# lukecq1231/nats

Measured on AMD Instinct MI355X. Metric: train_tokens_per_sec, higher is better.
Workload: dtype bf16; 1 GPU; model=distraction-gru-seq2seq, dim=1000, dim_word=100, enc_depth=1, dim_att=100, vocab=30000, src_len=800, tgt_len=100, batch_per_gpu=20, global_batch=20, seq_len=800, optimizer=adadelta+clip100, parallelism=dp1, step_graph=False

## Files before the change

### nats_amd/ops/hip/cond_gru.hip

```cpp

#include <torch/extension.h>
#include <ATen/cuda/CUDAContext.h>

#include <algorithm>

#include "common.h"
#include "gru_kernels.h"

namespace {

__global__ void cond_small_gemm_bt(const bf16_t* __restrict__ A,
                                   const bf16_t* __restrict__ Bt,
                                   float* __restrict__ Cpart, int B, int N,
                                   int ldK, int Kpad) {
  const int m0 = blockIdx.x * 16;
  const int n0 = blockIdx.y * 16;
  const int KS = gridDim.z;
  const int kchunk = ((Kpad / KS + 31) / 32) * 32;
  const int kbeg = min(Kpad, (int)blockIdx.z * kchunk);
  const int kend = min(Kpad, kbeg + kchunk);
  f32x4 acc = {0.f, 0.f, 0.f, 0.f};
  NATS_MFMA_KLOOP(acc, A, m0, ldK, Bt, n0, Kpad, kbeg, kend);
  const int lane = threadIdx.x & (NATS_WAVE - 1);
  const int col = n0 + (lane & 15);
  const int rbase = m0 + (lane >> 4) * 4;
  if (col >= N) return;
  float* C = Cpart + (long)blockIdx.z * 32 * N;
#pragma unroll
  for (int i = 0; i < 4; ++i) {
    const int row = rbase + i;
    if (row < B) C[(long)row * N + col] = acc[i];
  }
}

__global__ __launch_bounds__(256) void cond_attn_escore(
    const float* __restrict__ pctx,
    const float* __restrict__ ps_part,
    int PS_KS,
    const float* __restrict__ accA,
    const float* __restrict__ Dwei,
    const float* __restrict__ Uatt,
    const float* __restrict__ catt_p,
    float* __restrict__ e_buf,
    int B, int Ts, int A) {
  extern __shared__ float sm_e[];
  float* sm_ps = sm_e;
  float* sm_dw = sm_e + A;
  float* sm_ua = sm_e + 2 * A;
  const int b = blockIdx.x;
  for (int i = threadIdx.x; i < A; i += blockDim.x) {
    float ps = 0.f;
    for (int k = 0; k < PS_KS; ++k) ps += ps_part[((long)k * 32 + b) * A + i];
    sm_ps[i] = ps;
    sm_dw[i] = Dwei[i];
    sm_ua[i] = Uatt[i];
  }
  __syncthreads();
  const int s = blockIdx.y * blockDim.x + threadIdx.x;
  if (s >= Ts) return;
  const int ACH = gridDim.z;
  const int chunkA = ((A + ACH - 1) / ACH + 3) & ~3;
  const int ibeg = blockIdx.z * chunkA;
  const int iend = min(A, ibeg + chunkA);
  if (ibeg >= iend) return;
  const float accAu = accA[(long)b * Ts + s];
  const float* prow = pctx + ((long)s * B + b) * A;
  float e = (blockIdx.z == 0) ? catt_p[0] : 0.f;
  for (int i = ibeg; i < iend; ++i) {
    e += tanhf(prow[i] + sm_ps[i] + accAu * sm_dw[i]) * sm_ua[i];
  }
  if (ACH == 1) {
    e_buf[(long)s * B + b] += e;
  } else {
    atomicAdd(e_buf + (long)s * B + b, e);
  }
}

__global__ __launch_bounds__(1024) void cond_attn_softmax(
    float* __restrict__ accA,
    float* __restrict__ accA_used_t,
    const float* __restrict__ ctx_mask,
    const float* __restrict__ mask_t,
    float* __restrict__ e_buf,
    float* __restrict__ alphas_t,
    const float* __restrict__ ps_part,
    int PS_KS,
    float* __restrict__ pstate_t,
    int A,
    int B, int Ts) {
  {
    const int b0 = blockIdx.x;
    for (int i = threadIdx.x; i < A; i += blockDim.x) {
      float ps = 0.f;
      for (int k = 0; k < PS_KS; ++k)
        ps += ps_part[((long)k * 32 + b0) * A + i];
      pstate_t[(long)b0 * A + i] = ps;
    }
  }
  const int b = blockIdx.x;

  float lmax = -INFINITY;
  for (int s = threadIdx.x; s < Ts; s += blockDim.x) {
    if (ctx_mask != nullptr && ctx_mask[(long)s * B + b] == 0.f) continue;
    lmax = fmaxf(lmax, e_buf[(long)s * B + b]);
  }
  const float bmax = block_reduce_max(lmax);
  const float M = isfinite(bmax) ? bmax : 0.f;

  float lsum = 0.f;
  for (int s = threadIdx.x; s < Ts; s += blockDim.x) {
    float a = __expf(e_buf[(long)s * B + b] - M);
    e_buf[(long)s * B + b] = 0.f;
    if (ctx_mask != nullptr) a *= ctx_mask[(long)s * B + b];
    alphas_t[(long)b * Ts + s] = a;
    lsum += a;
  }
  const float inv = 1.f / block_reduce_sum(lsum);

  const float mm = (mask_t != nullptr) ? mask_t[b] : 1.f;
  for (int s = threadIdx.x; s < Ts; s += blockDim.x) {
    const float al = alphas_t[(long)b * Ts + s] * inv;
    alphas_t[(long)b * Ts + s] = al;
    accA_used_t[(long)b * Ts + s] = accA[(long)b * Ts + s];
    accA[(long)b * Ts + s] += mm * al;
  }
}

__global__ void cond_attn_ctx_partial(
    const bf16_t* __restrict__ ctx_bf,
    const float* __restrict__ alphas_t,
    float* __restrict__ ctxpre_f32,
    int B, int Ts, int C, int SCH) {
  const int b = blockIdx.x;
  const int c = blockIdx.y * blockDim.x + threadIdx.x;
  if (c >= C) return;
  const int chunk = (Ts + SCH - 1) / SCH;
  const int sbeg = blockIdx.z * chunk;
  const int send = min(Ts, sbeg + chunk);
  float s0 = 0.f, s1 = 0.f, s2 = 0.f, s3 = 0.f;
  int s = sbeg;
  for (; s + 4 <= send; s += 4) {
    s0 += (float)ctx_bf[((long)(s + 0) * B + b) * C + c] *
          alphas_t[(long)b * Ts + s + 0];
    s1 += (float)ctx_bf[((long)(s + 1) * B + b) * C + c] *
          alphas_t[(long)b * Ts + s + 1];
    s2 += (float)ctx_bf[((long)(s + 2) * B + b) * C + c] *
          alphas_t[(long)b * Ts + s + 2];
    s3 += (float)ctx_bf[((long)(s + 3) * B + b) * C + c] *
          alphas_t[(long)b * Ts + s + 3];
  }
  for (; s < send; ++s)
    s0 += (float)ctx_bf[((long)s * B + b) * C + c] *
          alphas_t[(long)b * Ts + s];
  atomicAdd(&ctxpre_f32[(long)b * C + c], s0 + s1 + s2 + s3);
}

__global__ void cond_attn_gate_fwd(
    float* __restrict__ ctxpre_f32,
    const float* __restrict__ Ucon, const float* __restrict__ Wcon,
    float* __restrict__ accC,
    bf16_t* __restrict__ accC_used_t,
    bf16_t* __restrict__ ctxpre_t,
    float* __restrict__ ctxs_t,
    bf16_t* __restrict__ hc_bf,
    int ctx_off, int ldK1, const float* __restrict__ mask_t, int B, int C) {
  const int b = blockIdx.x;
  const int c = blockIdx.y * blockDim.x + threadIdx.x;
  if (c >= C) return;
  const float sum = ctxpre_f32[(long)b * C + c];
  ctxpre_f32[(long)b * C + c] = 0.f;
  ctxpre_t[(long)b * C + c] = (bf16_t)sum;
  const float accCv = accC[(long)b * C + c];
  accC_used_t[(long)b * C + c] = (bf16_t)accCv;
  const float g = tanhf(Ucon[c] * sum + accCv * Wcon[c]);
  ctxs_t[(long)b * C + c] = g;
  hc_bf[(long)b * ldK1 + ctx_off + c] = (bf16_t)g;
  const float mm = (mask_t != nullptr) ? mask_t[b] : 1.f;
  accC[(long)b * C + c] = accCv + mm * g;
}

__global__ __launch_bounds__(1024) void cond_gru1_step_fwd(
    const bf16_t* __restrict__ hc_bf,
    const float* __restrict__ h1_t,
    const bf16_t* __restrict__ W1pk,
    const float* __restrict__ b1,
    const float* __restrict__ bx1,
    const float* __restrict__ mask_t,
    float* __restrict__ h2_t,
    bf16_t* __restrict__ h2bf_out,
    int ld_h2bf,
    float* __restrict__ saved1_t,
    int B, int H, int K1) {
  __shared__ float pre[4][2][32][JB + 1];

  const int wg = blockIdx.x;
  const int wave = threadIdx.x / NATS_WAVE;
  const int m = wave / 8;
  const int g = (wave % 8) / 2;
  const int ks = wave % 2;
  const int j0 = wg * JB;
  const int khalf = ((K1 / 2 + 31) / 32) * 32;
  const int kbeg = ks * khalf;
  const int kend = min(K1, (ks + 1) * khalf);

  f32x4 acc = {0.f, 0.f, 0.f, 0.f};
  const bf16_t* brow = W1pk + (long)(wg * 4 + g) * JB * K1;
  NATS_MFMA_KLOOP(acc, hc_bf, 16 * m, K1, brow, 0, K1, kbeg, kend);
  store_cd_lds(pre[g][ks], acc, 16 * m);
  __syncthreads();

  for (int idx = threadIdx.x; idx < B * JB; idx += blockDim.x) {
    const int b = idx / JB;
    const int c = idx % JB;
    const int j = j0 + c;
    if (j >= H) continue;
    const float pxa = pre[2][0][b][c] + pre[2][1][b][c];
    const float pxb = pre[3][0][b][c] + pre[3][1][b][c];
    const GruCellFwd o = gru_cell_fwd(
        pre[0][0][b][c] + pre[0][1][b][c] + b1[j],
        pre[1][0][b][c] + pre[1][1][b][c] + b1[H + j], pxa + bx1[j], pxb,
        h1_t[(long)b * H + j], mask_t, b);
    h2_t[(long)b * H + j] = o.hnew;
    h2bf_out[(long)b * ld_h2bf + j] = (bf16_t)o.hnew;
    saved1_t[(long)b * 4 * H + j] = o.r;
    saved1_t[(long)b * 4 * H + H + j] = o.u;
    saved1_t[(long)b * 4 * H + 2 * H + j] = pxa;
    saved1_t[(long)b * 4 * H + 3 * H + j] = o.hbar;
  }
}

__global__ __launch_bounds__(1024) void cond_gru1_gemm_splitk(
    const bf16_t* __restrict__ hc_bf,
    const bf16_t* __restrict__ W1pk,
    float* __restrict__ part,
    int H, int K1, int Hpad) {
  __shared__ float pre[4][2][32][JB + 1];

  const int wg = blockIdx.x;
  const int ksb = blockIdx.y;
  const int KS = gridDim.y;
  const int wave = threadIdx.x / NATS_WAVE;
  const int m = wave / 8;
  const int g = (wave % 8) / 2;
  const int ks = wave % 2;
  const int j0 = wg * JB;
  const int nchunk = 2 * KS;
  const int kchunk = ((K1 / nchunk + 31) / 32) * 32;
  const int kidx = 2 * ksb + ks;
  const int kbeg = min(K1, kidx * kchunk);
  const int kend = min(K1, (kidx + 1) * kchunk);

  f32x4 acc = {0.f, 0.f, 0.f, 0.f};
  const bf16_t* brow = W1pk + (long)(wg * 4 + g) * JB * K1;
  NATS_MFMA_KLOOP(acc, hc_bf, 16 * m, K1, brow, 0, K1, kbeg, kend);
  store_cd_lds(pre[g][ks], acc, 16 * m);
  __syncthreads();

  float* dst = part + ((long)ksb * 4 + 0) * 32 * Hpad;
  for (int idx = threadIdx.x; idx < 4 * 32 * JB; idx += blockDim.x) {
    const int gg = idx / (32 * JB);
    const int b = (idx / JB) % 32;
    const int c = idx % JB;
    dst[((long)gg * 32 + b) * Hpad + j0 + c] =
        pre[gg][0][b][c] + pre[gg][1][b][c];
  }
}

__global__ void cond_gru1_step_pointwise(
    const float* __restrict__ part,
    int KS,
    const float* __restrict__ h1_t,
    const float* __restrict__ b1,
    const float* __restrict__ bx1,
    const float* __restrict__ mask_t,
    float* __restrict__ h2_t,
    bf16_t* __restrict__ h2bf_out,
    int ld_h2bf,
    float* __restrict__ saved1_t,
    int B, int H, int Hpad) {
  const long total = (long)B * H;
  for (long idx = blockIdx.x * blockDim.x + threadIdx.x; idx < total;
       idx += (long)gridDim.x * blockDim.x) {
    const int b = idx / H;
    const int j = idx % H;
    float p0 = 0.f, p1 = 0.f, p2 = 0.f, p3 = 0.f;
    const long bj = (long)b * Hpad + j;
    for (int k = 0; k < KS; ++k) {
      const float* pk = part + (long)k * 4 * 32 * Hpad;
      p0 += pk[bj];
      p1 += pk[(long)32 * Hpad + bj];
      p2 += pk[(long)2 * 32 * Hpad + bj];
      p3 += pk[(long)3 * 32 * Hpad + bj];
    }
    const float pxa = p2;
    const GruCellFwd o = gru_cell_fwd(p0 + b1[j], p1 + b1[H + j],
                                      pxa + bx1[j], p3, h1_t[idx], mask_t, b);
    h2_t[idx] = o.hnew;
    h2bf_out[(long)b * ld_h2bf + j] = (bf16_t)o.hnew;
    saved1_t[(long)b * 4 * H + j] = o.r;
    saved1_t[(long)b * 4 * H + H + j] = o.u;
    saved1_t[(long)b * 4 * H + 2 * H + j] = pxa;
    saved1_t[(long)b * 4 * H + 3 * H + j] = o.hbar;
  }
}


__global__ void cond_gru1_bwd_pointwise(
    const float* __restrict__ dh_carry,
    const float* __restrict__ dh_carry2,
    const float* __restrict__ dh2_all_t,
    const float* __restrict__ saved1_t,
    const float* __restrict__ h1_all_t,
    const float* __restrict__ bx1,
    const float* __restrict__ mask_t,
    bf16_t* __restrict__ dstep1,
    bf16_t* __restrict__ dstepC,
    int ldK3,
    float* __restrict__ ddirect_h1,
    bf16_t* __restrict__ dpre1_t,
    const float* __restrict__ dctxs_t,
    const float* __restrict__ daccC,
    float* __restrict__ dctx_dir,
    int C,
    float* __restrict__ dot_buf,
    int B, int H) {
  const long total = (long)B * H;
  const long total_all = total + (long)B * C + B;
  for (long idx2 = blockIdx.x * blockDim.x + threadIdx.x; idx2 < total_all;
       idx2 += (long)gridDim.x * blockDim.x) {
    if (idx2 >= total) {
      const long e = idx2 - total;
      if (e < (long)B * C) {
        const int b = e / C;
        const float mm = (mask_t != nullptr) ? mask_t[b] : 1.f;
        float v = mm * daccC[e];
        if (dctxs_t != nullptr) v += dctxs_t[e];
        dctx_dir[e] = v;
      } else {
        dot_buf[e - (long)B * C] = 0.f;
      }
      continue;
    }
    const long idx = idx2;
    const int b = idx / H;
    const int j = idx % H;
    float dh2 = dh_carry[idx];
    if (dh_carry2 != nullptr) dh2 += dh_carry2[idx];
    if (dh2_all_t != nullptr) dh2 += dh2_all_t[idx];
    const float r2 = saved1_t[(long)b * 4 * H + j];
    const float u2 = saved1_t[(long)b * 4 * H + H + j];
    const float pxa = saved1_t[(long)b * 4 * H + 2 * H + j];
    const float hbar = saved1_t[(long)b * 4 * H + 3 * H + j];
    const float h1v = h1_all_t[idx];
    const float mm = (mask_t != nullptr) ? mask_t[b] : 1.f;
    const GruCellBwd o =
        gru_cell_bwd(dh2, r2, u2, pxa + bx1[j], hbar, h1v, mm);
    ddirect_h1[idx] = o.ddirect;
    dstep1[(long)b * ldK3 + j] = (bf16_t)o.dpr;
    dstep1[(long)b * ldK3 + H + j] = (bf16_t)o.dpu;
    dstep1[(long)b * ldK3 + 2 * H + j] = (bf16_t)o.dpxl;
    dstepC[(long)b * ldK3 + j] = (bf16_t)o.dpr;
    dstepC[(long)b * ldK3 + H + j] = (bf16_t)o.dpu;
    dstepC[(long)b * ldK3 + 2 * H + j] = (bf16_t)o.dpx;
    dpre1_t[(long)b * 4 * H + j] = (bf16_t)o.dpr;
    dpre1_t[(long)b * 4 * H + H + j] = (bf16_t)o.dpu;
    dpre1_t[(long)b * 4 * H + 2 * H + j] = (bf16_t)o.dpx;
    dpre1_t[(long)b * 4 * H + 3 * H + j] = (bf16_t)o.dpxl;
  }
}

__global__ __launch_bounds__(384) void cond_bwd_gemm_dual_gate(
    const bf16_t* __restrict__ dstep1, const bf16_t* __restrict__ U1cat,
    const float* __restrict__ ddirect_h1, float* __restrict__ dh1_buf,
    int H, const bf16_t* __restrict__ dstepC,
    const bf16_t* __restrict__ W1cat, const float* __restrict__ dctx_dir,
    int C, int Kpad,
    const float* __restrict__ ctxs_t,
    const float* __restrict__ Ucon, const float* __restrict__ Wcon,
    float* __restrict__ daccC,
    float* __restrict__ dctxpre_f32,
    bf16_t* __restrict__ dctxpre_all_t,
    const bf16_t* __restrict__ ctxpre_t,
    const bf16_t* __restrict__ accC_used_t,
    float* __restrict__ gdUcon,
    float* __restrict__ gdWcon,
    int B) {
  __shared__ float ucon_s[JB], wcon_s[JB];
  __shared__ float part[3][32][JB + 1];
  const bool ctx_side = (blockIdx.y == 1);
  if (ctx_side && threadIdx.x < JB) {
    ucon_s[threadIdx.x] = 0.f;
    wcon_s[threadIdx.x] = 0.f;
  }
  const int N = ctx_side ? C : H;
  if ((int)blockIdx.x * JB >= N) return;
  const bf16_t* dstep = ctx_side ? dstepC : dstep1;
  const bf16_t* Wt = ctx_side ? W1cat : U1cat;

  const int wg = blockIdx.x;
  const int wave = threadIdx.x / NATS_WAVE;
  const int m = wave / 3;
  const int ks = wave % 3;
  const int i0 = wg * JB;
  const int kchunk = ((Kpad / 3 + 31) / 32) * 32;
  const int kbeg = ks * kchunk;
  const int kend = min(Kpad, (ks + 1) * kchunk);
  f32x4 acc = {0.f, 0.f, 0.f, 0.f};
  NATS_MFMA_KLOOP(acc, dstep, 16 * m, Kpad, Wt, i0, Kpad, kbeg, kend);
  store_cd_lds(part[ks], acc, 16 * m);
  __syncthreads();

  for (int idx = threadIdx.x; idx < B * JB; idx += blockDim.x) {
    const int b = idx / JB;
    const int cc = idx % JB;
    const int i = i0 + cc;
    if (i >= N) continue;
    const long bi = (long)b * N + i;
    const float sum = part[0][b][cc] + part[1][b][cc] + part[2][b][cc];
    if (!ctx_side) {
      dh1_buf[bi] = ddirect_h1[bi] + sum;
    } else {
      const float v = dctx_dir[bi] + sum;
      const float g = ctxs_t[bi];
      const float dg = v * (1.f - g * g);
      const float dpre = dg * Ucon[i];
      dctxpre_f32[bi] = dpre;
      dctxpre_all_t[bi] = (bf16_t)dpre;
      daccC[bi] += dg * Wcon[i];
      atomicAdd(ucon_s + cc, dg * (float)ctxpre_t[bi]);
      atomicAdd(wcon_s + cc, dg * (float)accC_used_t[bi]);
    }
  }
  if (ctx_side) {
    __syncthreads();
    if (threadIdx.x < JB && i0 + (int)threadIdx.x < N) {
      atomicAdd(gdUcon + i0 + threadIdx.x, ucon_s[threadIdx.x]);
      atomicAdd(gdWcon + i0 + threadIdx.x, wcon_s[threadIdx.x]);
    }
  }
}

__device__ __forceinline__ bf16x8 frag_a_f32pad(const float* A, int row0,
                                                int ld, int k0, int Rows,
                                                int Kcols) {
  const int lane = threadIdx.x & (NATS_WAVE - 1);
  const int r = row0 + (lane & 15);
  const int kb = k0 + (lane >> 4) * 8;
  bf16x8 v;
#pragma unroll
  for (int i = 0; i < 8; ++i) {
    const int k = kb + i;
    v[i] = (bf16_t)((r < Rows && k < Kcols) ? A[(long)r * ld + k] : 0.f);
  }
  return v;
}

__global__ __launch_bounds__(384) void cond_dh_carry_gemm_split(
    const bf16_t* __restrict__ dstep,
    const bf16_t* __restrict__ Wt,
    const float* __restrict__ ddirect,
    float* __restrict__ out,
    int B, int H, int Kpad) {
  __shared__ float part[3][32][JB + 1];
  const int wg = blockIdx.x;
  const int ks2 = blockIdx.y;
  const int wave = threadIdx.x / NATS_WAVE;
  const int m = wave / 3;
  const int ks = wave % 3;
  const int i0 = wg * JB;
  const int khalf = ((Kpad / 2 + 31) / 32) * 32;
  const int hbeg = min(Kpad, ks2 * khalf);
  const int hend = min(Kpad, hbeg + khalf);
  const int kchunk = (((hend - hbeg) / 3 + 31) / 32) * 32;
  const int kbeg = hbeg + ks * kchunk;
  const int kend = min(hend, kbeg + kchunk);
  f32x4 acc = {0.f, 0.f, 0.f, 0.f};
  NATS_MFMA_KLOOP(acc, dstep, 16 * m, Kpad, Wt, i0, Kpad, kbeg, kend);
  store_cd_lds(part[ks], acc, 16 * m);
  __syncthreads();
  float* o = out + (long)ks2 * B * H;
  for (int idx = threadIdx.x; idx < B * JB; idx += blockDim.x) {
    const int b = idx / JB;
    const int cc = idx % JB;
    const int i = i0 + cc;
    if (i >= H) continue;
    float v = part[0][b][cc] + part[1][b][cc] + part[2][b][cc];
    if (ks2 == 0) v += ddirect[(long)b * H + i];
    o[(long)b * H + i] = v;
  }
}

__global__ __launch_bounds__(384) void cond_dh1_att_gemm(
    const float* __restrict__ dpstate_t,
    const bf16_t* __restrict__ WattB,
    float* __restrict__ dh1_buf,
    int B, int H, int A, int Apad) {
  __shared__ float part[3][32][JB + 1];
  const int wg = blockIdx.x;
  const int wave = threadIdx.x / NATS_WAVE;
  const int m = wave / 3;
  const int ks = wave % 3;
  const int i0 = wg * JB;
  const int kchunk = ((Apad / 3 + 31) / 32) * 32;
  const int kbeg = ks * kchunk;
  const int kend = min(Apad, (ks + 1) * kchunk);
  f32x4 acc = {0.f, 0.f, 0.f, 0.f};
  for (int k = kbeg; k + 32 <= kend; k += 32) {
    bf16x8 a = frag_a_f32pad(dpstate_t, 16 * m, A, k, B, A);
    bf16x8 bfr = frag_bt_rowmajor(WattB, i0, Apad, k);
    acc = __builtin_amdgcn_mfma_f32_16x16x32_bf16(a, bfr, acc, 0, 0, 0);
  }
  store_cd_lds(part[ks], acc, 16 * m);
  __syncthreads();
  for (int idx = threadIdx.x; idx < B * JB; idx += blockDim.x) {
    const int b = idx / JB;
    const int cc = idx % JB;
    const int i = i0 + cc;
    if (i >= H) continue;
    dh1_buf[(long)b * H + i] +=
        part[0][b][cc] + part[1][b][cc] + part[2][b][cc];
  }
}

__global__ __launch_bounds__(256) void cond_attn_bwd_dalpha(
    const bf16_t* __restrict__ ctx_bf,
    const float* __restrict__ dctxpre_f32,
    const float* __restrict__ alphas_t,
    const float* __restrict__ daccA,
    const float* __restrict__ mask_t,
    const float* __restrict__ dalphas_t,
    float* __restrict__ dal_buf,
    float* __restrict__ dot_buf,
    int B, int Ts, int C) {
  const int b = blockIdx.x;
  const int wave = threadIdx.x / NATS_WAVE;
  const int lane = threadIdx.x & (NATS_WAVE - 1);
  const int s = blockIdx.y * 4 + wave;
  if (s >= Ts) return;
  const bf16_t* crow = ctx_bf + ((long)s * B + b) * C;
  const float* drow = dctxpre_f32 + (long)b * C;
  float part = 0.f;
  const int C8 = C & ~7;
  for (int c = lane * 8; c < C8; c += NATS_WAVE * 8) {
    bf16x8 v = *(const bf16x8*)(crow + c);
    const float4 d0 = *(const float4*)(drow + c);
    const float4 d1 = *(const float4*)(drow + c + 4);
    part += (float)v[0] * d0.x + (float)v[1] * d0.y + (float)v[2] * d0.z +
            (float)v[3] * d0.w + (float)v[4] * d1.x + (float)v[5] * d1.y +
            (float)v[6] * d1.z + (float)v[7] * d1.w;
  }
  for (int c = C8 + lane; c < C; c += NATS_WAVE) {
    part += (float)crow[c] * drow[c];
  }
#pragma unroll
  for (int off = NATS_WAVE / 2; off > 0; off >>= 1)
    part += __shfl_down(part, off);
  if (lane == 0) {
    float dal = part;
    const float mm = (mask_t != nullptr) ? mask_t[b] : 1.f;
    dal += mm * daccA[(long)b * Ts + s];
    if (dalphas_t != nullptr) dal += dalphas_t[(long)b * Ts + s];
    dal_buf[(long)s * B + b] = dal;
  }
}

__global__ __launch_bounds__(256) void cond_attn_bwd_dot(
    const float* __restrict__ alphas_t, const float* __restrict__ dal_buf,
    float* __restrict__ dot_buf, int B, int Ts) {
  const int b = blockIdx.x;
  float part = 0.f;
  for (int s = threadIdx.x; s < Ts; s += blockDim.x)
    part += alphas_t[(long)b * Ts + s] * dal_buf[(long)s * B + b];
  const float S = block_reduce_sum(part);
  if (threadIdx.x == 0) dot_buf[b] = S;
}

__global__ __launch_bounds__(256) void cond_attn_bwd_scatter(
    const float* __restrict__ alphas_t,
    const float* __restrict__ dal_buf,
    const float* __restrict__ dot_buf,
    const float* __restrict__ pctx,
    const float* __restrict__ pstate_t,
    const float* __restrict__ accA_used_t,
    const float* __restrict__ Dwei, const float* __restrict__ Uatt,
    float* __restrict__ daccA,
    float* __restrict__ dpctx_acc,
    float* __restrict__ pc_buf,
    int B, int Ts, int A, int Tpad8) {
  const int b = blockIdx.x;
  const int s = blockIdx.y * blockDim.x + threadIdx.x;
  if (s >= Ts) return;
  const int ACH = gridDim.z;
  const int chunkA = ((A + ACH - 1) / ACH + 3) & ~3;
  const int ibeg = blockIdx.z * chunkA;
  const int iend = min(A, ibeg + chunkA);
  if (ibeg >= iend) return;
  const float al = alphas_t[(long)b * Ts + s];
  const float de = al * (dal_buf[(long)s * B + b] - dot_buf[b]);
  const float accAu = accA_used_t[(long)b * Ts + s];
  const float* prow = pctx + ((long)s * B + b) * A;
  const float* srow = pstate_t + (long)b * A;
  float* dprow = dpctx_acc + ((long)s * B + b) * A;
  float daccA_add = 0.f;
  const int A4 = (A % 4 == 0) ? iend : ibeg;
  int i = ibeg;
  for (; i < A4; i += 4) {
    const float4 p = *(const float4*)(prow + i);
    const float4 st = *(const float4*)(srow + i);
    const float4 dw = *(const float4*)(Dwei + i);
    const float4 ua = *(const float4*)(Uatt + i);
    float4 dpv = *(const float4*)(dprow + i);
    const float pc0 = tanhf(p.x + st.x + accAu * dw.x);
    const float pc1 = tanhf(p.y + st.y + accAu * dw.y);
    const float pc2 = tanhf(p.z + st.z + accAu * dw.z);
    const float pc3 = tanhf(p.w + st.w + accAu * dw.w);
    const float d0 = de * (1.f - pc0 * pc0) * ua.x;
    const float d1 = de * (1.f - pc1 * pc1) * ua.y;
    const float d2 = de * (1.f - pc2 * pc2) * ua.z;
    const float d3 = de * (1.f - pc3 * pc3) * ua.w;
    dpv.x += d0;
    dpv.y += d1;
    dpv.z += d2;
    dpv.w += d3;
    *(float4*)(dprow + i) = dpv;
    daccA_add += d0 * dw.x + d1 * dw.y + d2 * dw.z + d3 * dw.w;
    pc_buf[((long)b * A + i) * Tpad8 + s] = pc0;
    pc_buf[((long)b * A + i + 1) * Tpad8 + s] = pc1;
    pc_buf[((long)b * A + i + 2) * Tpad8 + s] = pc2;
    pc_buf[((long)b * A + i + 3) * Tpad8 + s] = pc3;
  }
  for (; i < iend; ++i) {
    const float pc = tanhf(prow[i] + srow[i] + accAu * Dwei[i]);
    const float dpc = de * (1.f - pc * pc) * Uatt[i];
    dprow[i] += dpc;
    daccA_add += dpc * Dwei[i];
    pc_buf[((long)b * A + i) * Tpad8 + s] = pc;
  }
  if (ACH == 1) {
    daccA[(long)b * Ts + s] += daccA_add;
  } else {
    atomicAdd(daccA + (long)b * Ts + s, daccA_add);
  }
}

__global__ __launch_bounds__(256) void cond_attn_bwd_reduce(
    const float* __restrict__ alphas_t,
    const float* __restrict__ dal_buf,
    const float* __restrict__ dot_buf,
    const float* __restrict__ accA_used_t,
    const float* __restrict__ pc_buf,
    const float* __restrict__ Uatt,
    float* __restrict__ dpstate_t,
    float* __restrict__ gdDwei,
    float* __restrict__ gdUatt,
    float* __restrict__ gdcatt,
    int B, int Ts, int A, int Apad, int Tpad8, int SCH) {
  extern __shared__ __attribute__((aligned(16))) char smem_raw[];
  const int chunk = (Ts + SCH - 1) / SCH;
  float* sm_de = (float*)smem_raw;
  float* sm_au = sm_de + chunk;
  const int b = blockIdx.x;
  const int sbeg = blockIdx.y * chunk;
  const int send = min(Ts, sbeg + chunk);
  const float dot = dot_buf[b];
  float dc = 0.f;
  for (int s = sbeg + threadIdx.x; s < send; s += blockDim.x) {
    const float de = alphas_t[(long)b * Ts + s] *
                     (dal_buf[(long)s * B + b] - dot);
    sm_de[s - sbeg] = de;
    sm_au[s - sbeg] = accA_used_t[(long)b * Ts + s];
    dc += de;
  }
  const float dc_blk = block_reduce_sum(dc);
  if (threadIdx.x == 0) atomicAdd(gdcatt, dc_blk);
  for (int i = threadIdx.x; i < A; i += blockDim.x) {
    const float* prow = pc_buf + ((long)b * A + i) * Tpad8;
    const float ua = Uatt[i];
    float sps = 0.f, sdw = 0.f, sua = 0.f;
    int s = sbeg;
    const int a8beg = (sbeg + 7) & ~7;
    const int a8end = send & ~7;
    for (; s < min(a8beg, send); ++s) {
      const float pc = prow[s];
      const float de = sm_de[s - sbeg];
      const float dpc = de * (1.f - pc * pc) * ua;
      sps += dpc;
      sdw += dpc * sm_au[s - sbeg];
      sua += de * pc;
    }
    for (; s + 8 <= a8end; s += 8) {
      const float4 p0 = *(const float4*)(prow + s);
      const float4 p1 = *(const float4*)(prow + s + 4);
      const float pv[8] = {p0.x, p0.y, p0.z, p0.w, p1.x, p1.y, p1.z, p1.w};
#pragma unroll
      for (int k = 0; k < 8; ++k) {
        const float pc = pv[k];
        const float de = sm_de[s + k - sbeg];
        const float dpc = de * (1.f - pc * pc) * ua;
        sps += dpc;
        sdw += dpc * sm_au[s + k - sbeg];
        sua += de * pc;
      }
    }
    for (; s < send; ++s) {
      const float pc = prow[s];
      const float de = sm_de[s - sbeg];
      const float dpc = de * (1.f - pc * pc) * ua;
      sps += dpc;
      sdw += dpc * sm_au[s - sbeg];
      sua += de * pc;
    }
    atomicAdd(&dpstate_t[(long)b * A + i], sps);
    atomicAdd(&gdDwei[i], sdw);
    atomicAdd(&gdUatt[i], sua);
  }
}

}

std::vector<torch::Tensor> cond_gru_fwd(
    torch::Tensor yg, torch::Tensor yc, c10::optional<torch::Tensor> mask,
    torch::Tensor init_state, torch::Tensor ctx_bf,
    c10::optional<torch::Tensor> ctx_mask, torch::Tensor pctx,
    torch::Tensor Upk2, torch::Tensor W1pk, torch::Tensor WattPk,
    torch::Tensor b1, torch::Tensor bx1, torch::Tensor Uatt,
    torch::Tensor catt, torch::Tensor Dwei, torch::Tensor Wcon,
    torch::Tensor Ucon,
    c10::optional<torch::Tensor> accC0, c10::optional<torch::Tensor> accA0) {
  const int T = yg.size(0), B = yg.size(1);
  const int H = yc.size(2);
  const int Ts = ctx_bf.size(0), C = ctx_bf.size(2);
  const int A = Uatt.size(0);
  TORCH_CHECK(B <= 32, "cond_gru: batch must be <= 32");
  TORCH_CHECK(yg.dtype() == torch::kBFloat16 && yg.is_contiguous());
  TORCH_CHECK(ctx_bf.dtype() == torch::kBFloat16 && ctx_bf.is_contiguous());
  TORCH_CHECK(pctx.dtype() == torch::kFloat32 && pctx.is_contiguous());
  const int Hpad = Upk2.size(1);
  const int K1 = W1pk.size(1);
  const int ngrpH = cdiv(H, JB);
  TORCH_CHECK(Upk2.size(0) == ngrpH * 3 * JB);
  TORCH_CHECK(W1pk.size(0) == ngrpH * 4 * JB);

  auto optsF = yg.options().dtype(torch::kFloat32);
  auto optsB = yg.options();
  auto h2_all = torch::empty({T, B, H}, optsF);
  auto h1_all = torch::empty({T, B, H}, optsF);
  auto ctxs_all = torch::empty({T, B, C}, optsF);
  auto alphas_all = torch::empty({T, B, Ts}, optsF);
  auto saved2 = torch::empty({T, B, 3 * H}, optsB);
  auto saved1 = torch::empty({T, B, 4 * H}, optsF);
  auto pstate_all = torch::empty({T, B, A}, optsF);
  auto ctxpre_all = torch::empty({T, B, C}, optsB);
  auto accA_used = torch::empty({T, B, Ts}, optsF);
  auto accC_used = torch::empty({T, B, C}, optsB);
  auto accA = accA0.has_value() ? accA0->contiguous().to(torch::kFloat32)
                                : torch::zeros({B, Ts}, optsF);
  auto accC = accC0.has_value() ? accC0->contiguous().to(torch::kFloat32)
                                : torch::zeros({B, C}, optsF);
  auto h2bf = torch::zeros({2, 32, Hpad}, optsB);
  const int GRU1_KS = 4;
  auto gru1_part = torch::empty({GRU1_KS, 4, 32, Hpad}, optsF);
  const int GRU2_KS = 4;
  auto gru2_part = torch::empty({GRU2_KS, 3, 32, Hpad}, optsF);
  auto hc_bf = torch::zeros({32, K1}, optsB);
  auto e_buf = torch::zeros({Ts, B}, optsF);
  const int PS_KS = 4;
  auto ps_part = torch::empty({PS_KS, 32, A}, optsF);
  auto ctxpre_f32 = torch::zeros({B, C}, optsF);
  const int SCH = std::max(1, std::min(8, Ts / 64));
  auto init_f = init_state.contiguous().to(torch::kFloat32);
  h2bf[0].slice(0, 0, B).slice(1, 0, H).copy_(init_f.to(torch::kBFloat16));

  const OptF32 mask_f(mask), cmask_f(ctx_mask);
  const float* mask_p = mask_f.p;
  const float* cmask_p = cmask_f.p;

  auto stream = at::cuda::getCurrentCUDAStream().stream();
  const int Apad16 = cdiv(A, 16) * 16;
  const long hbstride = (long)32 * Hpad;
  bf16_t* h2bf_p = (bf16_t*)h2bf.data_ptr();

  for (int t = 0; t < T; ++t) {
    const float* h2prev = (t == 0)
                              ? init_f.data_ptr<float>()
                              : h2_all.data_ptr<float>() + (long)(t - 1) * B * H;
    const float* mt = mask_p ? mask_p + (long)t * B : nullptr;
    if (Hpad >= 1024) {
      hipLaunchKernelGGL(nats_gru2_gemm_splitk, dim3(ngrpH, GRU2_KS),
                         dim3(384), 0, stream, h2bf_p + (t % 2) * hbstride,
                         (const bf16_t*)Upk2.data_ptr(),
                         gru2_part.data_ptr<float>(), Hpad);
      hipLaunchKernelGGL(nats_gru2_step_pointwise, dim3(cdiv(B * H, 256)),
                         dim3(256), 0, stream, gru2_part.data_ptr<float>(),
                         GRU2_KS, h2prev,
                         (const bf16_t*)yg.data_ptr() + (long)t * B * 2 * H,
                         (const bf16_t*)yc.data_ptr() + (long)t * B * H, mt,
                         h1_all.data_ptr<float>() + (long)t * B * H,
                         (bf16_t*)hc_bf.data_ptr(), K1,
                         (bf16_t*)saved2.data_ptr() + (long)t * B * 3 * H, B,
                         H, Hpad);
    } else {
      hipLaunchKernelGGL(nats_gru_step_fwd, dim3(ngrpH), dim3(384), 0, stream,
                         h2bf_p + (t % 2) * hbstride, h2prev,
                         (const bf16_t*)Upk2.data_ptr(),
                         (const bf16_t*)yg.data_ptr() + (long)t * B * 2 * H,
                         (const bf16_t*)yc.data_ptr() + (long)t * B * H, mt,
                         h1_all.data_ptr<float>() + (long)t * B * H,
                         (bf16_t*)hc_bf.data_ptr(), K1,
                         (bf16_t*)saved2.data_ptr() + (long)t * B * 3 * H, B,
                         H, Hpad);
    }
    hipLaunchKernelGGL(cond_small_gemm_bt, dim3(2, Apad16 / 16, PS_KS),
                       dim3(64), 0, stream, (const bf16_t*)hc_bf.data_ptr(),
                       (const bf16_t*)WattPk.data_ptr(),
                       ps_part.data_ptr<float>(), B, A, K1,
                       (int)WattPk.size(1));
    hipLaunchKernelGGL(cond_attn_escore,
                       dim3(B, cdiv(Ts, 256), A >= 16 ? 4 : 1), dim3(256),
                       3 * A * sizeof(float), stream, pctx.data_ptr<float>(),
                       ps_part.data_ptr<float>(), PS_KS,
                       accA.data_ptr<float>(), Dwei.data_ptr<float>(),
                       Uatt.data_ptr<float>(), catt.data_ptr<float>(),
                       e_buf.data_ptr<float>(), B, Ts, A);
    hipLaunchKernelGGL(cond_attn_softmax, dim3(B), dim3(1024), 0, stream,
                       accA.data_ptr<float>(),
                       accA_used.data_ptr<float>() + (long)t * B * Ts,
                       cmask_p, mt, e_buf.data_ptr<float>(),
                       alphas_all.data_ptr<float>() + (long)t * B * Ts,
                       ps_part.data_ptr<float>(), PS_KS,
                       pstate_all.data_ptr<float>() + (long)t * B * A, A, B,
                       Ts);
    hipLaunchKernelGGL(cond_attn_ctx_partial,
                       dim3(B, cdiv(C, 256), SCH), dim3(256), 0, stream,
                       (const bf16_t*)ctx_bf.data_ptr(),
                       alphas_all.data_ptr<float>() + (long)t * B * Ts,
                       ctxpre_f32.data_ptr<float>(), B, Ts, C, SCH);
    hipLaunchKernelGGL(cond_attn_gate_fwd, dim3(B, cdiv(C, 256)), dim3(256),
                       0, stream, ctxpre_f32.data_ptr<float>(),
                       Ucon.data_ptr<float>(), Wcon.data_ptr<float>(),
                       accC.data_ptr<float>(),
                       (bf16_t*)accC_used.data_ptr() + (long)t * B * C,
                       (bf16_t*)ctxpre_all.data_ptr() + (long)t * B * C,
                       ctxs_all.data_ptr<float>() + (long)t * B * C,
                       (bf16_t*)hc_bf.data_ptr(), Hpad, K1, mt, B, C);
    if (K1 >= 2048) {
      hipLaunchKernelGGL(cond_gru1_gemm_splitk, dim3(ngrpH, GRU1_KS),
                         dim3(1024), 0, stream,
                         (const bf16_t*)hc_bf.data_ptr(),
                         (const bf16_t*)W1pk.data_ptr(),
                         gru1_part.data_ptr<float>(), H, K1, Hpad);
      hipLaunchKernelGGL(cond_gru1_step_pointwise, dim3(cdiv(B * H, 256)),
                         dim3(256), 0, stream, gru1_part.data_ptr<float>(),
                         GRU1_KS, h1_all.data_ptr<float>() + (long)t * B * H,
                         b1.data_ptr<float>(), bx1.data_ptr<float>(), mt,
                         h2_all.data_ptr<float>() + (long)t * B * H,
                         h2bf_p + ((t + 1) % 2) * hbstride, Hpad,
                         saved1.data_ptr<float>() + (long)t * B * 4 * H, B,
                         H, Hpad);
    } else {
      hipLaunchKernelGGL(cond_gru1_step_fwd, dim3(ngrpH), dim3(1024), 0,
                         stream, (const bf16_t*)hc_bf.data_ptr(),
                         h1_all.data_ptr<float>() + (long)t * B * H,
                         (const bf16_t*)W1pk.data_ptr(), b1.data_ptr<float>(),
                         bx1.data_ptr<float>(), mt,
                         h2_all.data_ptr<float>() + (long)t * B * H,
                         h2bf_p + ((t + 1) % 2) * hbstride, Hpad,
                         saved1.data_ptr<float>() + (long)t * B * 4 * H, B,
                         H, K1);
    }
  }
  HIP_CHECK(hipGetLastError());
  return {h2_all, ctxs_all, alphas_all, accC, accA, h1_all, saved2, saved1,
          pstate_all, ctxpre_all, accA_used, accC_used};
}

std::vector<torch::Tensor> cond_gru_bwd(
    torch::Tensor dh2_all, c10::optional<torch::Tensor> dctxs_all,
    c10::optional<torch::Tensor> dalphas_all,
    c10::optional<torch::Tensor> daccC_f, c10::optional<torch::Tensor> daccA_f,
    torch::Tensor yc, torch::Tensor h1_all, torch::Tensor h2_all,
    torch::Tensor ctxs_all, torch::Tensor alphas_all, torch::Tensor saved2,
    torch::Tensor saved1, torch::Tensor pstate_all, torch::Tensor ctxpre_all,
    torch::Tensor accA_used, torch::Tensor accC_used, torch::Tensor ctx_bf,
    torch::Tensor pctx, torch::Tensor init_state,
    c10::optional<torch::Tensor> mask,
    torch::Tensor U1cat,
    torch::Tensor W1cat,
    torch::Tensor U2cat,
    torch::Tensor WattB,
    torch::Tensor bx1, torch::Tensor Dwei, torch::Tensor Uatt,
    torch::Tensor Ucon, torch::Tensor Wcon) {
  const int T = dh2_all.size(0), B = dh2_all.size(1), H = dh2_all.size(2);
  const int Ts = ctx_bf.size(0), C = ctx_bf.size(2);
  const int A = Uatt.size(0);
  const int K3Hpad = U1cat.size(1);
  const int Apad32 = WattB.size(1);
  const int ngrpH = cdiv(H, JB);
  const int ngrpC = cdiv(C, JB);

  auto optsF = dh2_all.options().dtype(torch::kFloat32);
  auto optsB = dh2_all.options().dtype(torch::kBFloat16);
  auto dpre1_all = torch::empty({T, B, 4 * H}, optsB);
  auto dpre2_all = torch::empty({T, B, 4 * H}, optsB);
  auto dctxpre_all = torch::empty({T, B, C}, optsB);
  auto gdUcon = torch::zeros({C}, optsF);
  auto gdWcon = torch::zeros({C}, optsF);
  auto dpstate_all = torch::zeros({T, B, A}, optsF);
  auto dpctx_acc = torch::zeros({Ts, B, A}, optsF);
  auto gdDwei = torch::zeros({A}, optsF);
  auto gdUatt = torch::zeros({A}, optsF);
  auto gdcatt = torch::zeros({1}, optsF);

  auto dh_carry = torch::zeros({2, B, H}, optsF);
  auto dh1_buf = torch::zeros({B, H}, optsF);
  auto ddirect_h1 = torch::empty({B, H}, optsF);
  auto ddirect2 = torch::empty({B, H}, optsF);
  auto dctx_dir = torch::empty({B, C}, optsF);
  auto dctxpre_f32 = torch::empty({B, C}, optsF);
  auto daccA = daccA_f.has_value() ? daccA_f->contiguous().to(torch::kFloat32)
                                   : torch::zeros({B, Ts}, optsF);
  auto daccC = daccC_f.has_value() ? daccC_f->contiguous().to(torch::kFloat32)
                                   : torch::zeros({B, C}, optsF);
  auto dal_buf = torch::empty({Ts, B}, optsF);
  auto dot_buf = torch::empty({B}, optsF);
  const int Tpad8 = (Ts + 7) / 8 * 8;
  auto pc_buf = torch::empty({B, A, Tpad8}, optsF);
  const int Apad = Apad32;
  auto dstep1 = torch::zeros({32, K3Hpad}, optsB);
  auto dstepC = torch::zeros({32, K3Hpad}, optsB);
  auto dstep2 = torch::zeros({32, K3Hpad}, optsB);
  auto init_f = init_state.contiguous().to(torch::kFloat32);

  const OptF32 mask_f(mask), dctxs_f(dctxs_all), dalpha_f(dalphas_all);
  const float* mask_all = mask_f.p;
  const float* dctxs_p = dctxs_f.p;
  const float* dalpha_p = dalpha_f.p;

  auto stream = at::cuda::getCurrentCUDAStream().stream();
  auto dh2_c = dh2_all.contiguous().to(torch::kFloat32);
  const int pwH = (int)std::min<long>(512, (((long)B * H) + 255) / 256);
  const int pwHC =
      (int)std::min<long>(512, (((long)B * (H + C) + B) + 255) / 256);

  for (int t = T - 1; t >= 0; --t) {
    const float* mt = mask_all ? mask_all + (long)t * B : nullptr;
    const float* h2prev =
        (t == 0) ? init_f.data_ptr<float>()
                 : h2_all.data_ptr<float>() + (long)(t - 1) * B * H;
    hipLaunchKernelGGL(cond_gru1_bwd_pointwise, dim3(pwHC), dim3(256), 0,
                       stream, dh_carry.data_ptr<float>(),
                       dh_carry.data_ptr<float>() + (long)B * H,
                       dh2_c.data_ptr<float>() + (long)t * B * H,
                       saved1.data_ptr<float>() + (long)t * B * 4 * H,
                       h1_all.data_ptr<float>() + (long)t * B * H,
                       bx1.data_ptr<float>(), mt,
                       (bf16_t*)dstep1.data_ptr(), (bf16_t*)dstepC.data_ptr(),
                       K3Hpad, ddirect_h1.data_ptr<float>(),
                       (bf16_t*)dpre1_all.data_ptr() + (long)t * B * 4 * H,
                       dctxs_p ? dctxs_p + (long)t * B * C : nullptr,
                       daccC.data_ptr<float>(), dctx_dir.data_ptr<float>(), C,
                       dot_buf.data_ptr<float>(), B, H);
    hipLaunchKernelGGL(cond_bwd_gemm_dual_gate,
                       dim3(std::max(ngrpH, ngrpC), 2), dim3(384), 0, stream,
                       (const bf16_t*)dstep1.data_ptr(),
                       (const bf16_t*)U1cat.data_ptr(),
                       ddirect_h1.data_ptr<float>(),
                       dh1_buf.data_ptr<float>(), H,
                       (const bf16_t*)dstepC.data_ptr(),
                       (const bf16_t*)W1cat.data_ptr(),
                       dctx_dir.data_ptr<float>(), C, K3Hpad,
                       ctxs_all.data_ptr<float>() + (long)t * B * C,
                       Ucon.data_ptr<float>(), Wcon.data_ptr<float>(),
                       daccC.data_ptr<float>(), dctxpre_f32.data_ptr<float>(),
                       (bf16_t*)dctxpre_all.data_ptr() + (long)t * B * C,
                       (const bf16_t*)ctxpre_all.data_ptr() + (long)t * B * C,
                       (const bf16_t*)accC_used.data_ptr() + (long)t * B * C,
                       gdUcon.data_ptr<float>(), gdWcon.data_ptr<float>(),
                       B);
    hipLaunchKernelGGL(cond_attn_bwd_dalpha, dim3(B, cdiv(Ts, 4)),
                       dim3(256), 0, stream,
                       (const bf16_t*)ctx_bf.data_ptr(),
                       dctxpre_f32.data_ptr<float>(),
                       alphas_all.data_ptr<float>() + (long)t * B * Ts,
                       daccA.data_ptr<float>(), mt,
                       dalpha_p ? dalpha_p + (long)t * B * Ts : nullptr,
                       dal_buf.data_ptr<float>(), dot_buf.data_ptr<float>(),
                       B, Ts, C);
    hipLaunchKernelGGL(cond_attn_bwd_dot, dim3(B), dim3(256), 0, stream,
                       alphas_all.data_ptr<float>() + (long)t * B * Ts,
                       dal_buf.data_ptr<float>(), dot_buf.data_ptr<float>(),
                       B, Ts);
    hipLaunchKernelGGL(cond_attn_bwd_scatter,
                       dim3(B, cdiv(Ts, 256), A >= 32 ? 8 : (A >= 16 ? 4 : 1)),
                       dim3(256), 0, stream,
                       alphas_all.data_ptr<float>() + (long)t * B * Ts,
                       dal_buf.data_ptr<float>(), dot_buf.data_ptr<float>(),
                       pctx.data_ptr<float>(),
                       pstate_all.data_ptr<float>() + (long)t * B * A,
                       accA_used.data_ptr<float>() + (long)t * B * Ts,
                       Dwei.data_ptr<float>(), Uatt.data_ptr<float>(),
                       daccA.data_ptr<float>(), dpctx_acc.data_ptr<float>(),
                       pc_buf.data_ptr<float>(), B, Ts, A, Tpad8);
    const int RSCH = std::max(1, std::min(12, Ts / 64));
    hipLaunchKernelGGL(cond_attn_bwd_reduce, dim3(B, RSCH), dim3(256),
                       2 * ((Ts + RSCH - 1) / RSCH) * sizeof(float), stream,
                       alphas_all.data_ptr<float>() + (long)t * B * Ts,
                       dal_buf.data_ptr<float>(), dot_buf.data_ptr<float>(),
                       accA_used.data_ptr<float>() + (long)t * B * Ts,
                       pc_buf.data_ptr<float>(),
                       Uatt.data_ptr<float>(),
                       dpstate_all.data_ptr<float>() + (long)t * B * A,
                       gdDwei.data_ptr<float>(), gdUatt.data_ptr<float>(),
                       gdcatt.data_ptr<float>(), B, Ts, A, Apad32, Tpad8,
                       RSCH);
    hipLaunchKernelGGL(cond_dh1_att_gemm, dim3(ngrpH), dim3(384), 0, stream,
                       dpstate_all.data_ptr<float>() + (long)t * B * A,
                       (const bf16_t*)WattB.data_ptr(),
                       dh1_buf.data_ptr<float>(), B, H, A, Apad32);
    hipLaunchKernelGGL(nats_gru_step_bwd_pointwise, dim3(pwH), dim3(256), 0,
                       stream, dh1_buf.data_ptr<float>(), nullptr,
                       (const bf16_t*)saved2.data_ptr() + (long)t * B * 3 * H,
                       (const bf16_t*)yc.data_ptr() + (long)t * B * H, h2prev,
                       mt, (bf16_t*)dstep2.data_ptr(), K3Hpad,
                       ddirect2.data_ptr<float>(),
                       (bf16_t*)dpre2_all.data_ptr() + (long)t * B * 4 * H, B,
                       H);
    hipLaunchKernelGGL(cond_dh_carry_gemm_split, dim3(ngrpH, 2), dim3(384),
                       0, stream, (const bf16_t*)dstep2.data_ptr(),
                       (const bf16_t*)U2cat.data_ptr(),
                       ddirect2.data_ptr<float>(), dh_carry.data_ptr<float>(),
                       B, H, K3Hpad);
  }
  HIP_CHECK(hipGetLastError());
  auto dh_carry_sum = dh_carry[0] + dh_carry[1];
  return {dpre1_all, dpre2_all, dctxpre_all, gdUcon, dpstate_all,
          dpctx_acc, gdDwei, gdUatt, gdcatt, dh_carry_sum, daccC, daccA,
          gdWcon};
}
```

Before: 479,000 tokens/s.

## Fuse chunked online-softmax attention in forward and backward of conditional GRU

Forward attention (score, softmax, context weighted sum) is restructured into per-chunk kernels that compute local max/sum statistics and partial context sums. A combine kernel then rescales these and applies the gate, replacing four launches and global atomics per decoder step. Backward fuses the dot, scatter and reduce attention kernels into one chunked kernel that keeps pctx tiles in LDS and writes per-block gradient slots, which are summed once at the end. This cuts launch count and the pc_buf round trip, in exchange for more LDS pressure and partial-sum buffers.

```diff
diff --git a/nats_amd/ops/hip/cond_gru.hip b/nats_amd/ops/hip/cond_gru.hip
--- a/nats_amd/ops/hip/cond_gru.hip
+++ b/nats_amd/ops/hip/cond_gru.hip
@@ -33,7 +33,36 @@
   }
 }
 
-__global__ __launch_bounds__(256) void cond_attn_escore(
+constexpr int ATT_CH_MAX = 64;
+constexpr int ATT_THREADS = 256;
+
+static inline int attn_chunk_len(int B, int Ts) {
+  const long per = ((long)B * Ts + 255) / 256;
+  const int ch = (int)std::min<long>(ATT_CH_MAX, std::max<long>(16, per));
+  return (ch + 7) & ~7;
+}
+
+static inline int attn_lanes_per_s(int CH) {
+  int lps = 4;
+  while (lps < 16 && CH * lps * 2 <= ATT_THREADS) lps *= 2;
+  return lps;
+}
+
+__device__ __forceinline__ void attn_stage_vectors(
+    float* sm, const float* __restrict__ ps_part, int PS_KS, long ks_stride,
+    int b, const float* __restrict__ Dwei, const float* __restrict__ Uatt,
+    int A) {
+  for (int i = threadIdx.x; i < A; i += blockDim.x) {
+    float ps = 0.f;
+    for (int k = 0; k < PS_KS; ++k)
+      ps += ps_part[(long)k * ks_stride + (long)b * A + i];
+    sm[i] = ps;
+    sm[A + i] = Dwei[i];
+    sm[2 * A + i] = Uatt[i];
+  }
+}
+
+__global__ __launch_bounds__(ATT_THREADS) void cond_attn_fwd_chunk(
     const float* __restrict__ pctx,
     const float* __restrict__ ps_part,
     int PS_KS,
@@ -41,122 +70,133 @@
     const float* __restrict__ Dwei,
     const float* __restrict__ Uatt,
     const float* __restrict__ catt_p,
-    float* __restrict__ e_buf,
-    int B, int Ts, int A) {
-  extern __shared__ float sm_e[];
-  float* sm_ps = sm_e;
-  float* sm_dw = sm_e + A;
-  float* sm_ua = sm_e + 2 * A;
+    const float* __restrict__ ctx_mask,
+    const bf16_t* __restrict__ ctx_bf,
+    float* __restrict__ alphas_t,
+    float* __restrict__ stats,
+    float* __restrict__ ctx_part,
+    int B, int Ts, int A, int C, int CH, int lps) {
+  extern __shared__ __attribute__((aligned(16))) float sm_att[];
+  __shared__ float sm_e[ATT_CH_MAX];
+  __shared__ float sm_p[ATT_CH_MAX];
+  const float* sm_ps = sm_att;
+  const float* sm_dw = sm_att + A;
+  const float* sm_ua = sm_att + 2 * A;
   const int b = blockIdx.x;
-  for (int i = threadIdx.x; i < A; i += blockDim.x) {
-    float ps = 0.f;
-    for (int k = 0; k < PS_KS; ++k) ps += ps_part[((long)k * 32 + b) * A + i];
-    sm_ps[i] = ps;
-    sm_dw[i] = Dwei[i];
-    sm_ua[i] = Uatt[i];
-  }
+  const int NCH = gridDim.y;
+  const int sbeg = blockIdx.y * CH;
+  const int n = min(CH, Ts - sbeg);
+  attn_stage_vectors(sm_att, ps_part, PS_KS, (long)32 * A, b, Dwei, Uatt, A);
   __syncthreads();
-  const int s = blockIdx.y * blockDim.x + threadIdx.x;
-  if (s >= Ts) return;
-  const int ACH = gridDim.z;
-  const int chunkA = ((A + ACH - 1) / ACH + 3) & ~3;
-  const int ibeg = blockIdx.z * chunkA;
-  const int iend = min(A, ibeg + chunkA);
-  if (ibeg >= iend) return;
-  const float accAu = accA[(long)b * Ts + s];
-  const float* prow = pctx + ((long)s * B + b) * A;
-  float e = (blockIdx.z == 0) ? catt_p[0] : 0.f;
-  for (int i = ibeg; i < iend; ++i) {
-    e += tanhf(prow[i] + sm_ps[i] + accAu * sm_dw[i]) * sm_ua[i];
-  }
-  if (ACH == 1) {
-    e_buf[(long)s * B + b] += e;
-  } else {
-    atomicAdd(e_buf + (long)s * B + b, e);
-  }
-}
-
-__global__ __launch_bounds__(1024) void cond_attn_softmax(
+
+  const int gl = threadIdx.x % lps;
+  const int ngrp = ATT_THREADS / lps;
+  for (int ls = threadIdx.x / lps; ls < n; ls += ngrp) {
+    const int s = sbeg + ls;
+    const bool live =
+        (ctx_mask == nullptr) || ctx_mask[(long)s * B + b] != 0.f;
+    float e = 0.f;
+    if (live) {
+      const float accAu = accA[(long)b * Ts + s];
+      const float* prow = pctx + ((long)s * B + b) * A;
+      if (A % 4 == 0) {
+        for (int i = gl * 4; i < A; i += lps * 4) {
+          const float4 p = *(const float4*)(prow + i);
+          const float4 st = *(const float4*)(sm_ps + i);
+          const float4 dw = *(const float4*)(sm_dw + i);
+          const float4 ua = *(const float4*)(sm_ua + i);
+          e += tanhf(p.x + st.x + accAu * dw.x) * ua.x +
+               tanhf(p.y + st.y + accAu * dw.y) * ua.y +
+               tanhf(p.z + st.z + accAu * dw.z) * ua.z +
+               tanhf(p.w + st.w + accAu * dw.w) * ua.w;
+        }
+      } else {
+        for (int i = gl; i < A; i += lps)
+          e += tanhf(prow[i] + sm_ps[i] + accAu * sm_dw[i]) * sm_ua[i];
+      }
+    }
+    for (int off = lps / 2; off > 0; off >>= 1) e += __shfl_xor(e, off);
+    if (gl == 0) sm_e[ls] = live ? e + catt_p[0] : -INFINITY;
+  }
+  __syncthreads();
+
+  if (threadIdx.x < NATS_WAVE) {
+    const int ls = threadIdx.x;
+    const float e = (ls < n) ? sm_e[ls] : -INFINITY;
+    float m = e;
+#pragma unroll
+    for (int off = NATS_WAVE / 2; off > 0; off >>= 1)
+      m = fmaxf(m, __shfl_xor(m, off));
+    float p = 0.f;
+    if (e != -INFINITY) {
+      p = __expf(e - m);
+      if (ctx_mask != nullptr) p *= ctx_mask[(long)(sbeg + ls) * B + b];
+    }
+    float l = p;
+#pragma unroll
+    for (int off = NATS_WAVE / 2; off > 0; off >>= 1) l += __shfl_xor(l, off);
+    sm_p[ls] = p;
+    if (ls < n) alphas_t[(long)b * Ts + sbeg + ls] = p;
+    if (ls == 0) {
+      stats[((long)b * NCH + blockIdx.y) * 2] = m;
+      stats[((long)b * NCH + blockIdx.y) * 2 + 1] = l;
+    }
+  }
+  __syncthreads();
+
+  float* part = ctx_part + ((long)b * NCH + blockIdx.y) * C;
+  const long sstride = (long)B * C;
+  const bf16_t* cbase = ctx_bf + ((long)sbeg * B + b) * C;
+  const int C8 = C & ~7;
+  for (int c0 = threadIdx.x * 8; c0 < C8; c0 += ATT_THREADS * 8) {
+    float acc[8] = {0.f, 0.f, 0.f, 0.f, 0.f, 0.f, 0.f, 0.f};
+    const bf16_t* col = cbase + c0;
+    int ls = 0;
+    for (; ls + 8 <= n; ls += 8) {
+      bf16x8 v[8];
+#pragma unroll
+      for (int u = 0; u < 8; ++u)
+        v[u] = *(const bf16x8*)(col + (long)(ls + u) * sstride);
+#pragma unroll
+      for (int u = 0; u < 8; ++u) {
+        const float p = sm_p[ls + u];
+#pragma unroll
+        for (int k = 0; k < 8; ++k) acc[k] += (float)v[u][k] * p;
+      }
+    }
+    for (; ls < n; ++ls) {
+      const bf16x8 v = *(const bf16x8*)(col + (long)ls * sstride);
+      const float p = sm_p[ls];
+#pragma unroll
+      for (int k = 0; k < 8; ++k) acc[k] += (float)v[k] * p;
+    }
+    if (C % 4 == 0) {
+      *(float4*)(part + c0) = make_float4(acc[0], acc[1], acc[2], acc[3]);
+      *(float4*)(part + c0 + 4) = make_float4(acc[4], acc[5], acc[6], acc[7]);
+    } else {
+#pragma unroll
+      for (int k = 0; k < 8; ++k) part[c0 + k] = acc[k];
+    }
+  }
+  for (int c = C8 + threadIdx.x; c < C; c += ATT_THREADS) {
+    float acc = 0.f;
+    for (int ls = 0; ls < n; ++ls)
+      acc += (float)cbase[(long)ls * sstride + c] * sm_p[ls];
+    part[c] = acc;
+  }
+}
+
+__global__ __launch_bounds__(ATT_THREADS) void cond_attn_combine_gate(
+    const float* __restrict__ stats,
+    const float* __restrict__ ctx_part,
+    int NCH, int CH,
+    float* __restrict__ alphas_t,
     float* __restrict__ accA,
     float* __restrict__ accA_used_t,
-    const float* __restrict__ ctx_mask,
-    const float* __restrict__ mask_t,
-    float* __restrict__ e_buf,
-    float* __restrict__ alphas_t,
     const float* __restrict__ ps_part,
     int PS_KS,
     float* __restrict__ pstate_t,
-    int A,
-    int B, int Ts) {
-  {
-    const int b0 = blockIdx.x;
-    for (int i = threadIdx.x; i < A; i += blockDim.x) {
-      float ps = 0.f;
-      for (int k = 0; k < PS_KS; ++k)
-        ps += ps_part[((long)k * 32 + b0) * A + i];
-      pstate_t[(long)b0 * A + i] = ps;
-    }
-  }
-  const int b = blockIdx.x;
-
-  float lmax = -INFINITY;
-  for (int s = threadIdx.x; s < Ts; s += blockDim.x) {
-    if (ctx_mask != nullptr && ctx_mask[(long)s * B + b] == 0.f) continue;
-    lmax = fmaxf(lmax, e_buf[(long)s * B + b]);
-  }
-  const float bmax = block_reduce_max(lmax);
-  const float M = isfinite(bmax) ? bmax : 0.f;
-
-  float lsum = 0.f;
-  for (int s = threadIdx.x; s < Ts; s += blockDim.x) {
-    float a = __expf(e_buf[(long)s * B + b] - M);
-    e_buf[(long)s * B + b] = 0.f;
-    if (ctx_mask != nullptr) a *= ctx_mask[(long)s * B + b];
-    alphas_t[(long)b * Ts + s] = a;
-    lsum += a;
-  }
-  const float inv = 1.f / block_reduce_sum(lsum);
-
-  const float mm = (mask_t != nullptr) ? mask_t[b] : 1.f;
-  for (int s = threadIdx.x; s < Ts; s += blockDim.x) {
-    const float al = alphas_t[(long)b * Ts + s] * inv;
-    alphas_t[(long)b * Ts + s] = al;
-    accA_used_t[(long)b * Ts + s] = accA[(long)b * Ts + s];
-    accA[(long)b * Ts + s] += mm * al;
-  }
-}
-
-__global__ void cond_attn_ctx_partial(
-    const bf16_t* __restrict__ ctx_bf,
-    const float* __restrict__ alphas_t,
-    float* __restrict__ ctxpre_f32,
-    int B, int Ts, int C, int SCH) {
-  const int b = blockIdx.x;
-  const int c = blockIdx.y * blockDim.x + threadIdx.x;
-  if (c >= C) return;
-  const int chunk = (Ts + SCH - 1) / SCH;
-  const int sbeg = blockIdx.z * chunk;
-  const int send = min(Ts, sbeg + chunk);
-  float s0 = 0.f, s1 = 0.f, s2 = 0.f, s3 = 0.f;
-  int s = sbeg;
-  for (; s + 4 <= send; s += 4) {
-    s0 += (float)ctx_bf[((long)(s + 0) * B + b) * C + c] *
-          alphas_t[(long)b * Ts + s + 0];
-    s1 += (float)ctx_bf[((long)(s + 1) * B + b) * C + c] *
-          alphas_t[(long)b * Ts + s + 1];
-    s2 += (float)ctx_bf[((long)(s + 2) * B + b) * C + c] *
-          alphas_t[(long)b * Ts + s + 2];
-    s3 += (float)ctx_bf[((long)(s + 3) * B + b) * C + c] *
-          alphas_t[(long)b * Ts + s + 3];
-  }
-  for (; s < send; ++s)
-    s0 += (float)ctx_bf[((long)s * B + b) * C + c] *
-          alphas_t[(long)b * Ts + s];
-  atomicAdd(&ctxpre_f32[(long)b * C + c], s0 + s1 + s2 + s3);
-}
-
-__global__ void cond_attn_gate_fwd(
-    float* __restrict__ ctxpre_f32,
+    int A, int Ts,
     const float* __restrict__ Ucon, const float* __restrict__ Wcon,
     float* __restrict__ accC,
     bf16_t* __restrict__ accC_used_t,
@@ -164,19 +204,54 @@
     float* __restrict__ ctxs_t,
     bf16_t* __restrict__ hc_bf,
     int ctx_off, int ldK1, const float* __restrict__ mask_t, int B, int C) {
+  extern __shared__ float sm_w[];
   const int b = blockIdx.x;
+  const float* st = stats + (long)b * NCH * 2;
+  float M = -INFINITY;
+  for (int k = 0; k < NCH; ++k) M = fmaxf(M, st[2 * k]);
+  float L = 0.f;
+  for (int k = 0; k < NCH; ++k) {
+    const float l = st[2 * k + 1];
+    if (l > 0.f) L += l * __expf(st[2 * k] - M);
+  }
+  const float inv = (L > 0.f) ? 1.f / L : 0.f;
+  for (int k = threadIdx.x; k < NCH; k += blockDim.x)
+    sm_w[k] = (st[2 * k + 1] > 0.f) ? __expf(st[2 * k] - M) * inv : 0.f;
+  __syncthreads();
+  const float mm = (mask_t != nullptr) ? mask_t[b] : 1.f;
+
   const int c = blockIdx.y * blockDim.x + threadIdx.x;
-  if (c >= C) return;
-  const float sum = ctxpre_f32[(long)b * C + c];
-  ctxpre_f32[(long)b * C + c] = 0.f;
-  ctxpre_t[(long)b * C + c] = (bf16_t)sum;
-  const float accCv = accC[(long)b * C + c];
-  accC_used_t[(long)b * C + c] = (bf16_t)accCv;
-  const float g = tanhf(Ucon[c] * sum + accCv * Wcon[c]);
-  ctxs_t[(long)b * C + c] = g;
-  hc_bf[(long)b * ldK1 + ctx_off + c] = (bf16_t)g;
-  const float mm = (mask_t != nullptr) ? mask_t[b] : 1.f;
-  accC[(long)b * C + c] = accCv + mm * g;
+  if (c < C) {
+    const float* part = ctx_part + (long)b * NCH * C + c;
+    float sum = 0.f;
+#pragma unroll 4
+    for (int k = 0; k < NCH; ++k) sum += sm_w[k] * part[(long)k * C];
+    ctxpre_t[(long)b * C + c] = (bf16_t)sum;
+    const float accCv = accC[(long)b * C + c];
+    accC_used_t[(long)b * C + c] = (bf16_t)accCv;
+    const float g = tanhf(Ucon[c] * sum + accCv * Wcon[c]);
+    ctxs_t[(long)b * C + c] = g;
+    hc_bf[(long)b * ldK1 + ctx_off + c] = (bf16_t)g;
+    accC[(long)b * C + c] = accCv + mm * g;
+  }
+
+  const int sper = (Ts + gridDim.y - 1) / gridDim.y;
+  const int s0 = blockIdx.y * sper;
+  const int s1 = min(Ts, s0 + sper);
+  for (int s = s0 + threadIdx.x; s < s1; s += blockDim.x) {
+    const float al = alphas_t[(long)b * Ts + s] * sm_w[s / CH];
+    alphas_t[(long)b * Ts + s] = al;
+    const float av = accA[(long)b * Ts + s];
+    accA_used_t[(long)b * Ts + s] = av;
+    accA[(long)b * Ts + s] = av + mm * al;
+  }
+  if (blockIdx.y == 0) {
+    for (int i = threadIdx.x; i < A; i += blockDim.x) {
+      float ps = 0.f;
+      for (int k = 0; k < PS_KS; ++k) ps += ps_part[((long)k * 32 + b) * A + i];
+      pstate_t[(long)b * A + i] = ps;
+    }
+  }
 }
 
 __global__ __launch_bounds__(1024) void cond_gru1_step_fwd(
@@ -321,24 +396,18 @@
     const float* __restrict__ dctxs_t,
     const float* __restrict__ daccC,
     float* __restrict__ dctx_dir,
-    int C,
-    float* __restrict__ dot_buf,
-    int B, int H) {
+    int C, int B, int H) {
   const long total = (long)B * H;
-  const long total_all = total + (long)B * C + B;
+  const long total_all = total + (long)B * C;
   for (long idx2 = blockIdx.x * blockDim.x + threadIdx.x; idx2 < total_all;
        idx2 += (long)gridDim.x * blockDim.x) {
     if (idx2 >= total) {
       const long e = idx2 - total;
-      if (e < (long)B * C) {
-        const int b = e / C;
-        const float mm = (mask_t != nullptr) ? mask_t[b] : 1.f;
-        float v = mm * daccC[e];
-        if (dctxs_t != nullptr) v += dctxs_t[e];
-        dctx_dir[e] = v;
-      } else {
-        dot_buf[e - (long)B * C] = 0.f;
-      }
+      const int b = e / C;
+      const float mm = (mask_t != nullptr) ? mask_t[b] : 1.f;
+      float v = mm * daccC[e];
+      if (dctxs_t != nullptr) v += dctxs_t[e];
+      dctx_dir[e] = v;
       continue;
     }
     const long idx = idx2;
@@ -530,7 +599,6 @@
     const float* __restrict__ mask_t,
     const float* __restrict__ dalphas_t,
     float* __restrict__ dal_buf,
-    float* __restrict__ dot_buf,
     int B, int Ts, int C) {
   const int b = blockIdx.x;
   const int wave = threadIdx.x / NATS_WAVE;
@@ -560,160 +628,125 @@
     const float mm = (mask_t != nullptr) ? mask_t[b] : 1.f;
     dal += mm * daccA[(long)b * Ts + s];
     if (dalphas_t != nullptr) dal += dalphas_t[(long)b * Ts + s];
-    dal_buf[(long)s * B + b] = dal;
-  }
-}
-
-__global__ __launch_bounds__(256) void cond_attn_bwd_dot(
-    const float* __restrict__ alphas_t, const float* __restrict__ dal_buf,
-    float* __restrict__ dot_buf, int B, int Ts) {
-  const int b = blockIdx.x;
-  float part = 0.f;
-  for (int s = threadIdx.x; s < Ts; s += blockDim.x)
-    part += alphas_t[(long)b * Ts + s] * dal_buf[(long)s * B + b];
-  const float S = block_reduce_sum(part);
-  if (threadIdx.x == 0) dot_buf[b] = S;
-}
-
-__global__ __launch_bounds__(256) void cond_attn_bwd_scatter(
+    dal_buf[(long)b * Ts + s] = dal;
+  }
+}
+
+__global__ __launch_bounds__(ATT_THREADS) void cond_attn_bwd_fused(
     const float* __restrict__ alphas_t,
     const float* __restrict__ dal_buf,
-    const float* __restrict__ dot_buf,
     const float* __restrict__ pctx,
     const float* __restrict__ pstate_t,
     const float* __restrict__ accA_used_t,
     const float* __restrict__ Dwei, const float* __restrict__ Uatt,
     float* __restrict__ daccA,
     float* __restrict__ dpctx_acc,
-    float* __restrict__ pc_buf,
-    int B, int Ts, int A, int Tpad8) {
+    float* __restrict__ dpstate_t,
+    float* __restrict__ gslot,
+    int B, int Ts, int A, int CH, int lps) {
+  extern __shared__ __attribute__((aligned(16))) float sm_att[];
+  __shared__ float sm_de[ATT_CH_MAX];
+  __shared__ float sm_au[ATT_CH_MAX];
+  const int A4 = (A + 3) & ~3;
+  const float* sm_ps = sm_att;
+  const float* sm_dw = sm_att + A;
+  const float* sm_ua = sm_att + 2 * A;
+  float* t_dpc = sm_att + 3 * A4;
+  float* t_pc = t_dpc + (long)CH * A;
   const int b = blockIdx.x;
-  const int s = blockIdx.y * blockDim.x + threadIdx.x;
-  if (s >= Ts) return;
-  const int ACH = gridDim.z;
-  const int chunkA = ((A + ACH - 1) / ACH + 3) & ~3;
-  const int ibeg = blockIdx.z * chunkA;
-  const int iend = min(A, ibeg + chunkA);
-  if (ibeg >= iend) return;
-  const float al = alphas_t[(long)b * Ts + s];
-  const float de = al * (dal_buf[(long)s * B + b] - dot_buf[b]);
-  const float accAu = accA_used_t[(long)b * Ts + s];
-  const float* prow = pctx + ((long)s * B + b) * A;
-  const float* srow = pstate_t + (long)b * A;
-  float* dprow = dpctx_acc + ((long)s * B + b) * A;
-  float daccA_add = 0.f;
-  const int A4 = (A % 4 == 0) ? iend : ibeg;
-  int i = ibeg;
-  for (; i < A4; i += 4) {
-    const float4 p = *(const float4*)(prow + i);
-    const float4 st = *(const float4*)(srow + i);
-    const float4 dw = *(const float4*)(Dwei + i);
-    const float4 ua = *(const float4*)(Uatt + i);
-    float4 dpv = *(const float4*)(dprow + i);
-    const float pc0 = tanhf(p.x + st.x + accAu * dw.x);
-    const float pc1 = tanhf(p.y + st.y + accAu * dw.y);
-    const float pc2 = tanhf(p.z + st.z + accAu * dw.z);
-    const float pc3 = tanhf(p.w + st.w + accAu * dw.w);
-    const float d0 = de * (1.f - pc0 * pc0) * ua.x;
-    const float d1 = de * (1.f - pc1 * pc1) * ua.y;
-    const float d2 = de * (1.f - pc2 * pc2) * ua.z;
-    const float d3 = de * (1.f - pc3 * pc3) * ua.w;
-    dpv.x += d0;
-    dpv.y += d1;
-    dpv.z += d2;
-    dpv.w += d3;
-    *(float4*)(dprow + i) = dpv;
-    daccA_add += d0 * dw.x + d1 * dw.y + d2 * dw.z + d3 * dw.w;
-    pc_buf[((long)b * A + i) * Tpad8 + s] = pc0;
-    pc_buf[((long)b * A + i + 1) * Tpad8 + s] = pc1;
-    pc_buf[((long)b * A + i + 2) * Tpad8 + s] = pc2;
-    pc_buf[((long)b * A + i + 3) * Tpad8 + s] = pc3;
-  }
-  for (; i < iend; ++i) {
-    const float pc = tanhf(prow[i] + srow[i] + accAu * Dwei[i]);
-    const float dpc = de * (1.f - pc * pc) * Uatt[i];
-    dprow[i] += dpc;
-    daccA_add += dpc * Dwei[i];
-    pc_buf[((long)b * A + i) * Tpad8 + s] = pc;
-  }
-  if (ACH == 1) {
-    daccA[(long)b * Ts + s] += daccA_add;
-  } else {
-    atomicAdd(daccA + (long)b * Ts + s, daccA_add);
-  }
-}
-
-__global__ __launch_bounds__(256) void cond_attn_bwd_reduce(
-    const float* __restrict__ alphas_t,
-    const float* __restrict__ dal_buf,
-    const float* __restrict__ dot_buf,
-    const float* __restrict__ accA_used_t,
-    const float* __restrict__ pc_buf,
-    const float* __restrict__ Uatt,
-    float* __restrict__ dpstate_t,
-    float* __restrict__ gdDwei,
-    float* __restrict__ gdUatt,
-    float* __restrict__ gdcatt,
-    int B, int Ts, int A, int Apad, int Tpad8, int SCH) {
-  extern __shared__ __attribute__((aligned(16))) char smem_raw[];
-  const int chunk = (Ts + SCH - 1) / SCH;
-  float* sm_de = (float*)smem_raw;
-  float* sm_au = sm_de + chunk;
-  const int b = blockIdx.x;
-  const int sbeg = blockIdx.y * chunk;
-  const int send = min(Ts, sbeg + chunk);
-  const float dot = dot_buf[b];
+  const int NCH = gridDim.y;
+  const int sbeg = blockIdx.y * CH;
+  const int n = min(CH, Ts - sbeg);
+  attn_stage_vectors(sm_att, pstate_t, 1, 0, b, Dwei, Uatt, A);
+
+  float part = 0.f;
+  for (int s = threadIdx.x; s < Ts; s += blockDim.x)
+    part += alphas_t[(long)b * Ts + s] * dal_buf[(long)b * Ts + s];
+  const float dot = block_reduce_sum(part);
+
   float dc = 0.f;
-  for (int s = sbeg + threadIdx.x; s < send; s += blockDim.x) {
-    const float de = alphas_t[(long)b * Ts + s] *
-                     (dal_buf[(long)s * B + b] - dot);
-    sm_de[s - sbeg] = de;
-    sm_au[s - sbeg] = accA_used_t[(long)b * Ts + s];
-    dc += de;
-  }
-  const float dc_blk = block_reduce_sum(dc);
-  if (threadIdx.x == 0) atomicAdd(gdcatt, dc_blk);
+  if (threadIdx.x < NATS_WAVE) {
+    const int ls = threadIdx.x;
+    float de = 0.f, au = 0.f;
+    if (ls < n) {
+      const long bs = (long)b * Ts + sbeg + ls;
+      de = alphas_t[bs] * (dal_buf[bs] - dot);
+      au = accA_used_t[bs];
+    }
+    sm_de[ls] = de;
+    sm_au[ls] = au;
+    dc = de;
+#pragma unroll
+    for (int off = NATS_WAVE / 2; off > 0; off >>= 1)
+      dc += __shfl_xor(dc, off);
+  }
+  __syncthreads();
+
+  const int gl = threadIdx.x % lps;
+  const int ngrp = ATT_THREADS / lps;
+  for (int ls = threadIdx.x / lps; ls < n; ls += ngrp) {
+    const int s = sbeg + ls;
+    const float de = sm_de[ls];
+    const float accAu = sm_au[ls];
+    const float* prow = pctx + ((long)s * B + b) * A;
+    float* dprow = dpctx_acc + ((long)s * B + b) * A;
+    float* drow = t_dpc + (long)ls * A;
+    float* crow = t_pc + (long)ls * A;
+    float dacc = 0.f;
+    if (A % 4 == 0) {
+      for (int i = gl * 4; i < A; i += lps * 4) {
+        const float4 p = *(const float4*)(prow + i);
+        const float4 st = *(const float4*)(sm_ps + i);
+        const float4 dw = *(const float4*)(sm_dw + i);
+        const float4 ua = *(const float4*)(sm_ua + i);
+        float4 dpv = *(const float4*)(dprow + i);
+        float4 pc, d;
+        pc.x = tanhf(p.x + st.x + accAu * dw.x);
+        pc.y = tanhf(p.y + st.y + accAu * dw.y);
+        pc.z = tanhf(p.z + st.z + accAu * dw.z);
+        pc.w = tanhf(p.w + st.w + accAu * dw.w);
+        d.x = de * (1.f - pc.x * pc.x) * ua.x;
+        d.y = de * (1.f - pc.y * pc.y) * ua.y;
+        d.z = de * (1.f - pc.z * pc.z) * ua.z;
+        d.w = de * (1.f - pc.w * pc.w) * ua.w;
+        dpv.x += d.x;
+        dpv.y += d.y;
+        dpv.z += d.z;
+        dpv.w += d.w;
+        *(float4*)(dprow + i) = dpv;
+        dacc += d.x * dw.x + d.y * dw.y + d.z * dw.z + d.w * dw.w;
+        *(float4*)(drow + i) = d;
+        *(float4*)(crow + i) = pc;
+      }
+    } else {
+      for (int i = gl; i < A; i += lps) {
+        const float pc = tanhf(prow[i] + sm_ps[i] + accAu * sm_dw[i]);
+        const float d = de * (1.f - pc * pc) * sm_ua[i];
+        dprow[i] += d;
+        dacc += d * sm_dw[i];
+        drow[i] = d;
+        crow[i] = pc;
+      }
+    }
+    for (int off = lps / 2; off > 0; off >>= 1) dacc += __shfl_xor(dacc, off);
+    if (gl == 0) daccA[(long)b * Ts + s] += dacc;
+  }
+  __syncthreads();
+
+  float* slot = gslot + ((long)b * NCH + blockIdx.y) * (2 * A + 1);
   for (int i = threadIdx.x; i < A; i += blockDim.x) {
-    const float* prow = pc_buf + ((long)b * A + i) * Tpad8;
-    const float ua = Uatt[i];
     float sps = 0.f, sdw = 0.f, sua = 0.f;
-    int s = sbeg;
-    const int a8beg = (sbeg + 7) & ~7;
-    const int a8end = send & ~7;
-    for (; s < min(a8beg, send); ++s) {
-      const float pc = prow[s];
-      const float de = sm_de[s - sbeg];
-      const float dpc = de * (1.f - pc * pc) * ua;
-      sps += dpc;
-      sdw += dpc * sm_au[s - sbeg];
-      sua += de * pc;
-    }
-    for (; s + 8 <= a8end; s += 8) {
-      const float4 p0 = *(const float4*)(prow + s);
-      const float4 p1 = *(const float4*)(prow + s + 4);
-      const float pv[8] = {p0.x, p0.y, p0.z, p0.w, p1.x, p1.y, p1.z, p1.w};
-#pragma unroll
-      for (int k = 0; k < 8; ++k) {
-        const float pc = pv[k];
-        const float de = sm_de[s + k - sbeg];
-        const float dpc = de * (1.f - pc * pc) * ua;
-        sps += dpc;
-        sdw += dpc * sm_au[s + k - sbeg];
-        sua += de * pc;
-      }
-    }
-    for (; s < send; ++s) {
-      const float pc = prow[s];
-      const float de = sm_de[s - sbeg];
-      const float dpc = de * (1.f - pc * pc) * ua;
-      sps += dpc;
-      sdw += dpc * sm_au[s - sbeg];
-      sua += de * pc;
+    for (int ls = 0; ls < n; ++ls) {
+      const float d = t_dpc[(long)ls * A + i];
+      sps += d;
+      sdw += d * sm_au[ls];
+      sua += sm_de[ls] * t_pc[(long)ls * A + i];
     }
     atomicAdd(&dpstate_t[(long)b * A + i], sps);
-    atomicAdd(&gdDwei[i], sdw);
-    atomicAdd(&gdUatt[i], sua);
-  }
+    slot[i] += sdw;
+    slot[A + i] += sua;
+  }
+  if (threadIdx.x == 0) slot[2 * A] += dc;
 }
 
 }
@@ -763,11 +796,13 @@
   const int GRU2_KS = 4;
   auto gru2_part = torch::empty({GRU2_KS, 3, 32, Hpad}, optsF);
   auto hc_bf = torch::zeros({32, K1}, optsB);
-  auto e_buf = torch::zeros({Ts, B}, optsF);
   const int PS_KS = 4;
   auto ps_part = torch::empty({PS_KS, 32, A}, optsF);
-  auto ctxpre_f32 = torch::zeros({B, C}, optsF);
-  const int SCH = std::max(1, std::min(8, Ts / 64));
+  const int CH = attn_chunk_len(B, Ts);
+  const int NCH = cdiv(Ts, CH);
+  const int lps = attn_lanes_per_s(CH);
+  auto att_stats = torch::empty({B, NCH, 2}, optsF);
+  auto ctx_part = torch::empty({B, NCH, C}, optsF);
   auto init_f = init_state.contiguous().to(torch::kFloat32);
   h2bf[0].slice(0, 0, B).slice(1, 0, H).copy_(init_f.to(torch::kBFloat16));
 
@@ -815,28 +850,24 @@
                        (const bf16_t*)WattPk.data_ptr(),
                        ps_part.data_ptr<float>(), B, A, K1,
                        (int)WattPk.size(1));
-    hipLaunchKernelGGL(cond_attn_escore,
-                       dim3(B, cdiv(Ts, 256), A >= 16 ? 4 : 1), dim3(256),
+    hipLaunchKernelGGL(cond_attn_fwd_chunk, dim3(B, NCH), dim3(ATT_THREADS),
                        3 * A * sizeof(float), stream, pctx.data_ptr<float>(),
                        ps_part.data_ptr<float>(), PS_KS,
                        accA.data_ptr<float>(), Dwei.data_ptr<float>(),
                        Uatt.data_ptr<float>(), catt.data_ptr<float>(),
-                       e_buf.data_ptr<float>(), B, Ts, A);
-    hipLaunchKernelGGL(cond_attn_softmax, dim3(B), dim3(1024), 0, stream,
+                       cmask_p, (const bf16_t*)ctx_bf.data_ptr(),
+                       alphas_all.data_ptr<float>() + (long)t * B * Ts,
+                       att_stats.data_ptr<float>(),
+                       ctx_part.data_ptr<float>(), B, Ts, A, C, CH, lps);
+    hipLaunchKernelGGL(cond_attn_combine_gate, dim3(B, cdiv(C, ATT_THREADS)),
+                       dim3(ATT_THREADS), NCH * sizeof(float), stream,
+                       att_stats.data_ptr<float>(),
+                       ctx_part.data_ptr<float>(), NCH, CH,
+                       alphas_all.data_ptr<float>() + (long)t * B * Ts,
                        accA.data_ptr<float>(),
                        accA_used.data_ptr<float>() + (long)t * B * Ts,
-                       cmask_p, mt, e_buf.data_ptr<float>(),
-                       alphas_all.data_ptr<float>() + (long)t * B * Ts,
                        ps_part.data_ptr<float>(), PS_KS,
-                       pstate_all.data_ptr<float>() + (long)t * B * A, A, B,
-                       Ts);
-    hipLaunchKernelGGL(cond_attn_ctx_partial,
-                       dim3(B, cdiv(C, 256), SCH), dim3(256), 0, stream,
-                       (const bf16_t*)ctx_bf.data_ptr(),
-                       alphas_all.data_ptr<float>() + (long)t * B * Ts,
-                       ctxpre_f32.data_ptr<float>(), B, Ts, C, SCH);
-    hipLaunchKernelGGL(cond_attn_gate_fwd, dim3(B, cdiv(C, 256)), dim3(256),
-                       0, stream, ctxpre_f32.data_ptr<float>(),
+                       pstate_all.data_ptr<float>() + (long)t * B * A, A, Ts,
                        Ucon.data_ptr<float>(), Wcon.data_ptr<float>(),
                        accC.data_ptr<float>(),
                        (bf16_t*)accC_used.data_ptr() + (long)t * B * C,
@@ -907,9 +938,15 @@
   auto gdWcon = torch::zeros({C}, optsF);
   auto dpstate_all = torch::zeros({T, B, A}, optsF);
   auto dpctx_acc = torch::zeros({Ts, B, A}, optsF);
-  auto gdDwei = torch::zeros({A}, optsF);
-  auto gdUatt = torch::zeros({A}, optsF);
-  auto gdcatt = torch::zeros({1}, optsF);
+  const int A4 = (A + 3) & ~3;
+  const int lds_floats = 60 * 1024 / (int)sizeof(float);
+  TORCH_CHECK(3 * A4 + 2 * 8 * A <= lds_floats,
+              "cond_gru_bwd: dim_att too large for the attention tiles");
+  const int CH = std::min(attn_chunk_len(B, Ts),
+                          ((lds_floats - 3 * A4) / (2 * A)) & ~7);
+  const int NCH = cdiv(Ts, CH);
+  const int lps = attn_lanes_per_s(CH);
+  auto gslot = torch::zeros({B * NCH, 2 * A + 1}, optsF);
 
   auto dh_carry = torch::zeros({2, B, H}, optsF);
   auto dh1_buf = torch::zeros({B, H}, optsF);
@@ -921,11 +958,7 @@
                                    : torch::zeros({B, Ts}, optsF);
   auto daccC = daccC_f.has_value() ? daccC_f->contiguous().to(torch::kFloat32)
                                    : torch::zeros({B, C}, optsF);
-  auto dal_buf = torch::empty({Ts, B}, optsF);
-  auto dot_buf = torch::empty({B}, optsF);
-  const int Tpad8 = (Ts + 7) / 8 * 8;
-  auto pc_buf = torch::empty({B, A, Tpad8}, optsF);
-  const int Apad = Apad32;
+  auto dal_buf = torch::empty({B, Ts}, optsF);
   auto dstep1 = torch::zeros({32, K3Hpad}, optsB);
   auto dstepC = torch::zeros({32, K3Hpad}, optsB);
   auto dstep2 = torch::zeros({32, K3Hpad}, optsB);
@@ -940,7 +973,7 @@
   auto dh2_c = dh2_all.contiguous().to(torch::kFloat32);
   const int pwH = (int)std::min<long>(512, (((long)B * H) + 255) / 256);
   const int pwHC =
-      (int)std::min<long>(512, (((long)B * (H + C) + B) + 255) / 256);
+      (int)std::min<long>(512, (((long)B * (H + C)) + 255) / 256);
 
   for (int t = T - 1; t >= 0; --t) {
     const float* mt = mask_all ? mask_all + (long)t * B : nullptr;
@@ -959,7 +992,7 @@
                        (bf16_t*)dpre1_all.data_ptr() + (long)t * B * 4 * H,
                        dctxs_p ? dctxs_p + (long)t * B * C : nullptr,
                        daccC.data_ptr<float>(), dctx_dir.data_ptr<float>(), C,
-                       dot_buf.data_ptr<float>(), B, H);
+                       B, H);
     hipLaunchKernelGGL(cond_bwd_gemm_dual_gate,
                        dim3(std::max(ngrpH, ngrpC), 2), dim3(384), 0, stream,
                        (const bf16_t*)dstep1.data_ptr(),
@@ -984,35 +1017,17 @@
                        alphas_all.data_ptr<float>() + (long)t * B * Ts,
                        daccA.data_ptr<float>(), mt,
                        dalpha_p ? dalpha_p + (long)t * B * Ts : nullptr,
-                       dal_buf.data_ptr<float>(), dot_buf.data_ptr<float>(),
-                       B, Ts, C);
-    hipLaunchKernelGGL(cond_attn_bwd_dot, dim3(B), dim3(256), 0, stream,
+                       dal_buf.data_ptr<float>(), B, Ts, C);
+    hipLaunchKernelGGL(cond_attn_bwd_fused, dim3(B, NCH), dim3(ATT_THREADS),
+                       (3 * A4 + 2 * CH * A) * sizeof(float), stream,
                        alphas_all.data_ptr<float>() + (long)t * B * Ts,
-                       dal_buf.data_ptr<float>(), dot_buf.data_ptr<float>(),
-                       B, Ts);
-    hipLaunchKernelGGL(cond_attn_bwd_scatter,
-                       dim3(B, cdiv(Ts, 256), A >= 32 ? 8 : (A >= 16 ? 4 : 1)),
-                       dim3(256), 0, stream,
-                       alphas_all.data_ptr<float>() + (long)t * B * Ts,
-                       dal_buf.data_ptr<float>(), dot_buf.data_ptr<float>(),
-                       pctx.data_ptr<float>(),
+                       dal_buf.data_ptr<float>(), pctx.data_ptr<float>(),
                        pstate_all.data_ptr<float>() + (long)t * B * A,
                        accA_used.data_ptr<float>() + (long)t * B * Ts,
                        Dwei.data_ptr<float>(), Uatt.data_ptr<float>(),
                        daccA.data_ptr<float>(), dpctx_acc.data_ptr<float>(),
-                       pc_buf.data_ptr<float>(), B, Ts, A, Tpad8);
-    const int RSCH = std::max(1, std::min(12, Ts / 64));
-    hipLaunchKernelGGL(cond_attn_bwd_reduce, dim3(B, RSCH), dim3(256),
-                       2 * ((Ts + RSCH - 1) / RSCH) * sizeof(float), stream,
-                       alphas_all.data_ptr<float>() + (long)t * B * Ts,
-                       dal_buf.data_ptr<float>(), dot_buf.data_ptr<float>(),
-                       accA_used.data_ptr<float>() + (long)t * B * Ts,
-                       pc_buf.data_ptr<float>(),
-                       Uatt.data_ptr<float>(),
                        dpstate_all.data_ptr<float>() + (long)t * B * A,
-                       gdDwei.data_ptr<float>(), gdUatt.data_ptr<float>(),
-                       gdcatt.data_ptr<float>(), B, Ts, A, Apad32, Tpad8,
-                       RSCH);
+                       gslot.data_ptr<float>(), B, Ts, A, CH, lps);
     hipLaunchKernelGGL(cond_dh1_att_gemm, dim3(ngrpH), dim3(384), 0, stream,
                        dpstate_all.data_ptr<float>() + (long)t * B * A,
                        (const bf16_t*)WattB.data_ptr(),
@@ -1033,6 +1048,10 @@
   }
   HIP_CHECK(hipGetLastError());
   auto dh_carry_sum = dh_carry[0] + dh_carry[1];
+  auto gsum = gslot.sum(0);
+  auto gdDwei = gsum.slice(0, 0, A).contiguous();
+  auto gdUatt = gsum.slice(0, A, 2 * A).contiguous();
+  auto gdcatt = gsum.slice(0, 2 * A, 2 * A + 1).contiguous();
   return {dpre1_all, dpre2_all, dctxpre_all, gdUcon, dpstate_all,
           dpctx_acc, gdDwei, gdUatt, gdcatt, dh_carry_sum, daccC, daccA,
           gdWcon};
```

Measured after the change: 515,000 tokens/s, median of 6. +7.5%, better.
